# shivams15/navierstokessolver

Hardware: AMD Instinct MI355X
Metric: cell-updates/sec (MLUPS) + Poisson iters/sec, 4096^2 grid at 1/2/4/8 GPUs (higher is better)
Workload: dtype f64

## Files before the change

navierstokessolver_amd/csrc/ns_fps.hip:

```cpp
#include <hip/hip_ext.h>
#include <hip/hip_runtime.h>

#include <algorithm>

#include "ns_internal.h"

namespace nsg {

namespace {

struct cplx {
    double x, y;
};
__device__ inline cplx cadd(cplx a, cplx b) { return {a.x + b.x, a.y + b.y}; }
__device__ inline cplx csub(cplx a, cplx b) { return {a.x - b.x, a.y - b.y}; }
__device__ inline cplx cmul(cplx a, cplx b) { return {fma(a.x, b.x, -a.y * b.y), fma(a.x, b.y, a.y * b.x)}; }

__device__ inline double2 ld2(const double* p) { return *reinterpret_cast<const double2*>(p); }
__device__ inline void st2(double* p, double x, double y) { *reinterpret_cast<double2*>(p) = double2{x, y}; }

__device__ constexpr double C16[8] = {1.0, 0.92387953251128675613, 0.70710678118654752440, 0.38268343236508977173,
                                      0.0, -0.38268343236508977173, -0.70710678118654752440, -0.92387953251128675613};
__device__ constexpr double S16[8] = {0.0, 0.38268343236508977173, 0.70710678118654752440, 0.92387953251128675613,
                                      1.0, 0.92387953251128675613, 0.70710678118654752440, 0.38268343236508977173};
// ... 807 lines not shown
        } else {
#pragma unroll
            for (int q = 0; q < PT; q++) {
                const int k = tid + q * T;
                if (k < N) z[pz(k)] = cplx{ra[q], rb[q]};
            }
            __syncthreads();
            cplx v[PT];
#pragma unroll
            for (int q = 0; q < PT; q++) {
                const int k = tid + q * T;
                if (k < N) {
                    const cplx Xk = z[pz(k)];
                    const cplx Xn = k ? z[pz(N - k)] : cplx{0.0, 0.0};
                    v[q] = conjv(k, Xk.x, Xk.y, Xn.x, Xn.y);
                }
            }
            __syncthreads();
#pragma unroll
            for (int q = 0; q < PT; q++) {
                const int k = tid + q * T;
                if (k < N) z[pz(k)] = v[q];
            }
        }
        __syncthreads();
        fft_lds<LOGN>(z, tw, tid);
        if (PREF && p + (int)gridDim.x < npairs) load(p + gridDim.x);
        double* oa = out + (size_t)r0 * ld;
        double* ob = oa + ld;
#pragma unroll
        for (int q = 0; q < PT; q++) {
            const int j = tid + q * T;
            if (j < N) {
                const int n = (j & 1) ? N - 1 - (j >> 1) : (j >> 1);
                const cplx y = z[pz(n)];
                oa[j] = y.x * rn;
                if (two) ob[j] = -y.y * rn;
            }
        }
        __syncthreads();
    }
}


__device__ inline double piv_next(const FpsArgs& a, int gi, int k, double mu, double rprev, double pw, double pe,
                                  double pem, double& g) {
    const bool oe = a.outE && gi == a.nx - 1;
    g = (oe ? -0.5 * mu : pw) * rprev;
    const double p = fma(-g, pem, oe ? mu : -(pw + pe) + mu);
    return (a.pin && k == 0 && gi == a.nx - 1) ? 0.0 : 1.0 / p;
}


__device__ inline int fps_prow_block(const FpsArgs& a) {
    if (a.prowb) return a.prowb[blockIdx.x];
    return a.ptab && (int)(blockIdx.x * 128) >= a.kfast ? 0 : (1 << 30);
}
__device__ inline void piv_pair(const FpsArgs& a, bool fast, double2 pinf, int gi, int k0, const double (&mu)[2],
                                double (&r)[2], double pw, double pe, double pem, double& g0, double& g1, int pb) {
    if (fast && gi >= pb && gi != a.nx - 1) {
        g0 = pw * r[0];
        g1 = pw * r[1];
        const double2 t = a.ptab && gi < a.prow ? ld2(a.ptab + (size_t)gi * a.ld + k0) : pinf;
        r[0] = t.x;
        r[1] = t.y;
    } else {
        r[0] = piv_next(a, gi, k0, mu[0], r[0], pw, pe, pem, g0);
        r[1] = piv_next(a, gi, k0 + 1, mu[1], r[1], pw, pe, pem, g1);
    }
}

__device__ inline double mode0_shift(const FpsArgs& a, int k0, const double* f = nullptr) {
    if (k0 != 0) return 0.0;
    if (a.outE) return f && !a.s0_given ? 2.0 * f[(size_t)(a.nxl - 1) * a.ld] : *a.s0;
    return a.sh0 ? (a.sh0s != 0.0 ? a.sh0s : (double)a.ny) * *a.sh0 : 0.0;
}
__device__ inline double2 ldf0(const FpsArgs& a, const double* f, int li, int k0, double s0) {
    double2 x = ld2(f + (size_t)li * a.ld + k0);
    x.x -= s0;
    return x;
}

struct ChunkRows {
    double pw[FPS_M], pe[FPS_M], pem[FPS_M];
    __device__ inline void load(const FpsArgs& a, int li0, int rows) {
        (void)rows;
#pragma unroll
        for (int t = 0; t < FPS_M; t++) {
            const int gi = a.i0 + min(li0 + t, a.nxl - 1);
            pw[t] = a.pw[gi];
            pe[t] = a.pe[gi];
            const double pm = a.pe[max(gi - 1, 0)];
            pem[t] = gi > 0 ? pm : 0.0;
        }
    }
    __device__ inline void load_wave(const FpsArgs& a, int li0) {
        if constexpr (3 * FPS_M > 64) {
            load(a, li0, FPS_M);
            return;
        }
        const int lane = threadIdx.x & 63, t = lane % FPS_M, kind = lane / FPS_M;
        const int gi = a.i0 + min(li0 + t, a.nxl - 1);
        const int gk = kind == 2 ? max(gi - 1, 0) : gi;
        const double* src = kind == 0 ? a.pw : a.pe;
        double v = kind < 3 ? src[gk] : 0.0;
        if (kind == 2 && gi == 0) v = 0.0;
        const int lo = __double2loint(v), hi = __double2hiint(v);
        auto rd = [&](int l) {
            return __hiloint2double(__builtin_amdgcn_readlane(hi, l), __builtin_amdgcn_readlane(lo, l));
        };
#pragma unroll
        for (int q = 0; q < FPS_M; q++) {
            pw[q] = rd(q);
            pe[q] = rd(FPS_M + q);
            pem[q] = rd(2 * FPS_M + q);
        }
    }
};

__global__ void __launch_bounds__(64 * FPS_G) k_fps_t1(FpsArgs a, const double* __restrict__ f) {
    __shared__ double2 sE[FPS_G][64], sP[FPS_G][64];
    const int lane = threadIdx.x, w = __builtin_amdgcn_readfirstlane(threadIdx.y);
    const int k0 = 2 * (blockIdx.x * 64 + lane);
    const int grp = blockIdx.y, c = grp * FPS_G + w;
    const int li0 = c * FPS_M;
    const int rows = k0 < a.ny ? min(FPS_M, a.nxl - li0) : 0;
    double E[2] = {0.0, 0.0}, P[2] = {1.0, 1.0};
    if (rows > 0) {
        const double mu[2] = {a.mu[k0], a.mu[k0 + 1]};
        const double2 r0 = ld2(a.rp0 + (size_t)c * a.ld + k0);
        const double s0 = mode0_shift(a, k0);
        ChunkRows cr;
        cr.load(a, li0, rows);
        double2 fv[FPS_M];
#pragma unroll
        for (int t = 0; t < FPS_M; t++)
            if (t < rows) fv[t] = ldf0(a, f, li0 + t, k0, s0);
        double r[2] = {r0.x, r0.y};
#pragma unroll
        for (int t = 0; t < FPS_M; t++) {
            if (t < rows) {
                const int gi = a.i0 + li0 + t;
                const double fm[2] = {fv[t].x, fv[t].y};
#pragma unroll
                for (int m = 0; m < 2; m++) {
                    double g;
                    r[m] = piv_next(a, gi, k0 + m, mu[m], r[m], cr.pw[t], cr.pe[t], cr.pem[t], g);
                    E[m] = fma(-g, E[m], fm[m]);
                    P[m] = -g * P[m];
                }
            }
        }
        st2(a.ca + (size_t)c * a.ld + k0, E[0], E[1]);
        st2(a.ca + (size_t)(a.nch + c) * a.ld + k0, P[0], P[1]);
    }
    sE[w][lane] = double2{E[0], E[1]};
    sP[w][lane] = double2{P[0], P[1]};
    __syncthreads();
    if (w == 0 && k0 < a.ny) {
        double GE[2] = {0.0, 0.0}, GP[2] = {1.0, 1.0};
        for (int q = 0; q < FPS_G; q++) {
            const double2 e = sE[q][lane], pp = sP[q][lane];
            GE[0] = fma(pp.x, GE[0], e.x);
            GE[1] = fma(pp.y, GE[1], e.y);
            GP[0] = pp.x * GP[0];
            GP[1] = pp.y * GP[1];
        }
        st2(a.ga + (size_t)grp * a.ld + k0, GE[0], GE[1]);
        st2(a.ga + (size_t)(a.ngrp + grp) * a.ld + k0, GP[0], GP[1]);
    }
}
// ... 236 lines not shown
    const int li0 = c * FPS_M;
    const int rows = k0 < a.ny ? min(FPS_M, a.nxl - li0) : 0;
    double2 bx{0.0, 0.0}, br{1.0, 1.0};
    if (rows > 0) {
        bx = ld2(a.cb + (size_t)c * a.ld + k0);
        br = ld2(a.cb + (size_t)(a.nch + c) * a.ld + k0);
    }
    sX[w][lane] = bx;
    sR[w][lane] = br;
    __syncthreads();
    if (rows <= 0) return;
    ChunkRows cr;
    cr.load(a, li0, rows);
    double2 xv[FPS_M];
#pragma unroll
    for (int t = 0; t < FPS_M; t++)
        if (t < rows) xv[t] = ld2(f + (size_t)(li0 + t) * a.ld + k0);
    const double2 x0 = ld2(a.gx + (size_t)grp * a.ld + k0);
    double X[2] = {x0.x, x0.y};
    for (int q = FPS_G - 1; q > w; q--) {
        const double2 x = sX[q][lane], rr = sR[q][lane];
        X[0] = fma(rr.x, X[0], x.x);
        X[1] = fma(rr.y, X[1], x.y);
    }
    const double mu[2] = {a.mu[k0], a.mu[k0 + 1]};
    const double2 r0 = ld2(a.rp0 + (size_t)c * a.ld + k0);
    double r[2] = {r0.x, r0.y};
    double2 rv[FPS_M];
#pragma unroll
    for (int t = 0; t < FPS_M; t++) {
        if (t < rows) {
            const int gi = a.i0 + li0 + t;
            double g;
            r[0] = piv_next(a, gi, k0, mu[0], r[0], cr.pw[t], cr.pe[t], cr.pem[t], g);
            r[1] = piv_next(a, gi, k0 + 1, mu[1], r[1], cr.pw[t], cr.pe[t], cr.pem[t], g);
            rv[t] = double2{r[0], r[1]};
        }
    }
    double rho[2] = {1.0, 1.0};
#pragma unroll
    for (int t = FPS_M - 1; t >= 0; t--) {
        if (t < rows) {
            rho[0] = -cr.pe[t] * rv[t].x * rho[0];
            rho[1] = -cr.pe[t] * rv[t].y * rho[1];
            st2(f + (size_t)(li0 + t) * a.ld + k0, fma(rho[0], X[0], xv[t].x), fma(rho[1], X[1], xv[t].y));
        }
    }
}


__global__ void __launch_bounds__(64 * FPS_G) k_fps_t1b(FpsArgs a, const double* __restrict__ f) {
    __shared__ double2 sE[FPS_G][64], sP[FPS_G][64];
    const int lane = threadIdx.x, w = __builtin_amdgcn_readfirstlane(threadIdx.y);
    const int k0 = 2 * (blockIdx.x * 64 + lane);
    const int grp = FPS_SNAKE ? (int)gridDim.y - 1 - (int)blockIdx.y : (int)blockIdx.y, c = grp * FPS_G + w;
    const int li0 = c * FPS_M;
    const int rows = k0 < a.ny ? min(FPS_M, a.nxl - li0) : 0;
    double E[2] = {0.0, 0.0}, P[2] = {1.0, 1.0};
    ChunkRows cr;
    cr.load_wave(a, li0);
    if (rows > 0) {
        const double mu[2] = {a.mu[k0], a.mu[k0 + 1]};
        const double2 r0 = ld2(a.rp0 + (size_t)c * a.ld + k0);
        const double s0 = mode0_shift(a, k0, f);
        double2 yv[FPS_M], rv[FPS_M];
#pragma unroll
        for (int t = 0; t < FPS_M; t++)
            yv[t] = ldf0(a, f, min(li0 + t, a.nxl - 1), k0, s0);
        double r[2] = {r0.x, r0.y};
        const int pb = fps_prow_block(a);
        const bool fast = pb < a.nx;
        const double2 pinf = fast ? ld2(a.pinf + k0) : double2{0.0, 0.0};
#pragma unroll
        for (int t = 0; t < FPS_M; t++) {
            if (t < rows) {
                const int gi = a.i0 + li0 + t;
                double g0, g1;
                piv_pair(a, fast, pinf, gi, k0, mu, r, cr.pw[t], cr.pe[t], cr.pem[t], g0, g1, pb);
                E[0] = fma(-g0, E[0], yv[t].x);
                E[1] = fma(-g1, E[1], yv[t].y);
                P[0] = -g0 * P[0];
                P[1] = -g1 * P[1];
                yv[t] = double2{E[0], E[1]};
                rv[t] = double2{r[0], r[1]};
            }
        }
        double xl[2] = {0.0, 0.0};
#pragma unroll
        for (int t = FPS_M - 1; t >= 0; t--) {
            if (t < rows) {
                xl[0] = fma(yv[t].x, rv[t].x, -cr.pe[t] * rv[t].x * xl[0]);
                xl[1] = fma(yv[t].y, rv[t].y, -cr.pe[t] * rv[t].y * xl[1]);
            }
        }
        st2(a.ca + (size_t)c * a.ld + k0, E[0], E[1]);
        st2(a.ca + (size_t)(a.nch + c) * a.ld + k0, P[0], P[1]);
        st2(a.cb + (size_t)c * a.ld + k0, xl[0], xl[1]);
    }
    sE[w][lane] = double2{E[0], E[1]};
    sP[w][lane] = double2{P[0], P[1]};
    __syncthreads();
    if (w == 0 && k0 < a.ny) {
        double GE[2] = {0.0, 0.0}, GP[2] = {1.0, 1.0};
        for (int q = 0; q < FPS_G; q++) {
            const double2 e = sE[q][lane], pp = sP[q][lane];
            GE[0] = fma(pp.x, GE[0], e.x);
            GE[1] = fma(pp.y, GE[1], e.y);
            GP[0] = pp.x * GP[0];
            GP[1] = pp.y * GP[1];
        }
        st2(a.ga + (size_t)grp * a.ld + k0, GE[0], GE[1]);
        st2(a.ga + (size_t)(a.ngrp + grp) * a.ld + k0, GP[0], GP[1]);
    }
}

__global__ void __launch_bounds__(64) k_fps_mid(FpsArgs a, const double* __restrict__ f) {
    const int k0 = 2 * (blockIdx.x * 64 + threadIdx.x);
    const int grp = blockIdx.y;
    if (k0 >= a.ny) return;
    if (a.outE && !a.s0_given && k0 == 0 && grp == 0) *a.s0 = mode0_shift(a, 0, f);
    const double2 y0 = ld2(a.gc + (size_t)grp * a.ld + k0);
    double Y[2] = {y0.x, y0.y};
    double BX[FPS_G][2], BR[FPS_G][2];
    double2 le[FPS_G], lp[FPS_G], lb[FPS_G], lbe[FPS_G], lbr[FPS_G];
#pragma unroll
    for (int w = 0; w < FPS_G; w++) {
        const int c = min(grp * FPS_G + w, a.nch - 1);
        le[w] = ld2(a.ca + (size_t)c * a.ld + k0);
        lp[w] = ld2(a.ca + (size_t)(a.nch + c) * a.ld + k0);
        lb[w] = ld2(a.cb + (size_t)c * a.ld + k0);
        lbe[w] = ld2(a.bt + (size_t)c * a.ld + k0);
        lbr[w] = ld2(a.bt + (size_t)(a.nch + c) * a.ld + k0);
    }
#pragma unroll
    for (int w = 0; w < FPS_G; w++) {
        const int c = grp * FPS_G + w;
        BX[w][0] = BX[w][1] = 0.0;
        BR[w][0] = BR[w][1] = 1.0;
        if (c < a.nch) {
            double2 e = le[w];
            const double2 pp = lp[w];
            double2 bl = lb[w];
            if (a.m0e && k0 == 0) {
                const double sft = a.ny * *a.m0s;
                e.x -= sft * a.m0e[c];
                bl.x -= sft * a.m0b[c];
            }
            const double2 be = lbe[w], br = lbr[w];
            if (!a.mid_local) st2(a.ya + (size_t)c * a.ld + k0, Y[0], Y[1]);
            BX[w][0] = fma(be.x, Y[0], bl.x);
            BX[w][1] = fma(be.y, Y[1], bl.y);
            BR[w][0] = br.x;
            BR[w][1] = br.y;
            if (!a.mid_local) st2(a.cb + (size_t)c * a.ld + k0, BX[w][0], BX[w][1]);
            Y[0] = fma(pp.x, Y[0], e.x);
            Y[1] = fma(pp.y, Y[1], e.y);
        }
    }
    double GX[2] = {0.0, 0.0}, GR[2] = {1.0, 1.0};
#pragma unroll
    for (int w = FPS_G - 1; w >= 0; w--) {
        GX[0] = fma(BR[w][0], GX[0], BX[w][0]);
        GX[1] = fma(BR[w][1], GX[1], BX[w][1]);
        GR[0] = BR[w][0] * GR[0];
        GR[1] = BR[w][1] * GR[1];
    }
    st2(a.gb + (size_t)grp * a.ld + k0, GX[0], GX[1]);
    st2(a.gb + (size_t)(a.ngrp + grp) * a.ld + k0, GR[0], GR[1]);
}

constexpr int MS_MB = 16;
constexpr int MS_NT = 512;
template <int S, bool BACK, class LE, class LP, class SC>
__device__ __forceinline__ void ms_scan(int ngrp, int ny, int kb, int tid, LE ldE, LP ldP, SC stC, double (*sE)[MS_MB],
                                        double (*sP)[MS_MB], double (*sY)[MS_MB]) {
    const int lane = tid % MS_MB, s = tid / MS_MB;
    const int k = kb + lane;
    constexpr int B = 8;
    auto gq = [&](int q) { return BACK ? ngrp - 1 - q : q; };
    if (S > 1 && ngrp >= 2 * S) {
        const bool act = s < S && k < ny;
        const int per = (ngrp + S - 1) / S, q0 = s * per, q1 = min(ngrp, q0 + per);
        double AE = 0.0, AP = 1.0;
        if (act) {
            for (int qb = q0; qb < q1; qb += B) {
// ... 41 lines not shown
                    const int q = qb + t;
                    if (q < q1) {
                        stC(gq(q), lane, Y);
                        Y = fma(P[t], Y, E[t]);
                    }
                }
            }
        }
    } else if (s == 0 && k < ny) {
        double Y = 0.0;
        for (int q0 = 0; q0 < ngrp; q0 += B) {
            double E[B], P[B];
#pragma unroll
            for (int t = 0; t < B; t++) {
                const int q = q0 + t, qc = min(q, ngrp - 1);
                const double e = ldE(gq(qc), lane), pv = ldP(gq(qc), lane);
                E[t] = q < ngrp ? e : 0.0;
                P[t] = q < ngrp ? pv : 1.0;
            }
#pragma unroll
            for (int t = 0; t < B; t++) {
                const int q = q0 + t;
                if (q < ngrp) {
                    stC(gq(q), lane, Y);
                    Y = fma(P[t], Y, E[t]);
                }
            }
        }
    }
}
template <int S>
__global__ void __launch_bounds__(MS_NT) k_fps_midscan(FpsArgs a, const double* __restrict__ f) {
    extern __shared__ double ms_lds[];
    __shared__ double sE[S][MS_MB], sP[S][MS_MB], sY[S][MS_MB];
    static_assert(MS_NT >= S * MS_MB, "k_fps_midscan: a thread per mode and segment");
    const int tid = threadIdx.x, ngrp = a.ngrp, ld = a.ld, kb = blockIdx.x * MS_MB;
    double* gc = ms_lds;
    double* gbx = gc + (size_t)ngrp * MS_MB;
    double* gbr = gbx + (size_t)ngrp * MS_MB;
    ms_scan<S, false>(
        ngrp, a.ny, kb, tid, [&](int grp, int lane) { return a.ga[(size_t)grp * ld + kb + lane]; },
        [&](int grp, int lane) { return a.ga[(size_t)(ngrp + grp) * ld + kb + lane]; },
        [&](int grp, int lane, double Y) { gc[grp * MS_MB + lane] = Y; }, sE, sP, sY);
    __syncthreads();
    constexpr int NP = MS_MB / 2;
    for (int task = tid; task < NP * ngrp; task += MS_NT) {
        const int pr = task % NP, grp = task / NP;
        const int k0 = kb + 2 * pr;
        if (k0 >= a.ny) continue;
        if (a.outE && !a.s0_given && k0 == 0 && grp == 0) *a.s0 = mode0_shift(a, 0, f);
        double Y[2] = {gc[grp * MS_MB + 2 * pr], gc[grp * MS_MB + 2 * pr + 1]};
        double BX[FPS_G][2], BR[FPS_G][2];
        double2 le[FPS_G], lp[FPS_G], lb[FPS_G], lbe[FPS_G], lbr[FPS_G];
#pragma unroll
        for (int w = 0; w < FPS_G; w++) {
            const int c = min(grp * FPS_G + w, a.nch - 1);
            le[w] = ld2(a.ca + (size_t)c * a.ld + k0);
            lp[w] = ld2(a.ca + (size_t)(a.nch + c) * a.ld + k0);
            lb[w] = ld2(a.cb + (size_t)c * a.ld + k0);
            lbe[w] = ld2(a.bt + (size_t)c * a.ld + k0);
            lbr[w] = ld2(a.bt + (size_t)(a.nch + c) * a.ld + k0);
        }
#pragma unroll
        for (int w = 0; w < FPS_G; w++) {
            const int c = grp * FPS_G + w;
            BX[w][0] = BX[w][1] = 0.0;
            BR[w][0] = BR[w][1] = 1.0;
            if (c < a.nch) {
                double2 e = le[w];
                const double2 pp = lp[w];
                double2 bl = lb[w];
                if (a.m0e && k0 == 0) {
                    const double sft = a.ny * *a.m0s;
                    e.x -= sft * a.m0e[c];
                    bl.x -= sft * a.m0b[c];
                }
                const double2 be = lbe[w], br = lbr[w];
                st2(a.ya + (size_t)c * a.ld + k0, Y[0], Y[1]);
                BX[w][0] = fma(be.x, Y[0], bl.x);
                BX[w][1] = fma(be.y, Y[1], bl.y);
                BR[w][0] = br.x;
                BR[w][1] = br.y;
                st2(a.cb + (size_t)c * a.ld + k0, BX[w][0], BX[w][1]);
                Y[0] = fma(pp.x, Y[0], e.x);
                Y[1] = fma(pp.y, Y[1], e.y);
            }
        }
        double GX[2] = {0.0, 0.0}, GR[2] = {1.0, 1.0};
#pragma unroll
        for (int w = FPS_G - 1; w >= 0; w--) {
            GX[0] = fma(BR[w][0], GX[0], BX[w][0]);
            GX[1] = fma(BR[w][1], GX[1], BX[w][1]);
            GR[0] = BR[w][0] * GR[0];
            GR[1] = BR[w][1] * GR[1];
        }
        gbx[grp * MS_MB + 2 * pr] = GX[0];
        gbx[grp * MS_MB + 2 * pr + 1] = GX[1];
        gbr[grp * MS_MB + 2 * pr] = GR[0];
        gbr[grp * MS_MB + 2 * pr + 1] = GR[1];
    }
    __syncthreads();
    ms_scan<S, true>(
        ngrp, a.ny, kb, tid, [&](int grp, int lane) { return gbx[grp * MS_MB + lane]; },
        [&](int grp, int lane) { return gbr[grp * MS_MB + lane]; },
        [&](int grp, int lane, double Y) { a.gx[(size_t)grp * ld + kb + lane] = Y; }, sE, sP, sY);
}

template <bool GHOST>
__global__ void __launch_bounds__(64 * FPS_G) k_fps_t2b(FpsArgs a, double* __restrict__ f) {
    const int lane = threadIdx.x, w = __builtin_amdgcn_readfirstlane(threadIdx.y);
    const int k0 = 2 * (blockIdx.x * 64 + lane);
    const int grp = blockIdx.y, c = grp * FPS_G + w;
    const int li0 = c * FPS_M;
    const int rows = k0 < a.ny ? min(FPS_M, a.nxl - li0) : 0;
    ChunkRows cr;
    cr.load_wave(a, li0);
    if (rows <= 0) return;
    const double s0 = mode0_shift(a, k0);
    double2 yv[FPS_M];
#pragma unroll
    for (int t = 0; t < FPS_M; t++)
        yv[t] = ldf0(a, f, min(li0 + t, a.nxl - 1), k0, s0);
    const double2 yin = ld2(a.ya + (size_t)c * a.ld + k0);
    const double2 x0 = ld2(a.gx + (size_t)grp * a.ld + k0);
    double X[2] = {x0.x, x0.y};
    for (int q = FPS_G - 1; q > w; q--) {
        const int cq = grp * FPS_G + q;
        if (cq >= a.nch) continue;
        const double2 bx = ld2(a.cb + (size_t)cq * a.ld + k0), br = ld2(a.bt + (size_t)(a.nch + cq) * a.ld + k0);
        X[0] = fma(br.x, X[0], bx.x);
        X[1] = fma(br.y, X[1], bx.y);
    }
    if (GHOST && c == a.nch - 1 && a.i0 + a.nxl < a.nx) st2(f + (size_t)a.nxl * a.ld + k0, X[0], X[1]);
    const double mu[2] = {a.mu[k0], a.mu[k0 + 1]};
    const double2 r0 = ld2(a.rp0 + (size_t)c * a.ld + k0);
    double r[2] = {r0.x, r0.y}, y[2] = {yin.x, yin.y};
    double2 rv[FPS_M];
    const int pb = fps_prow_block(a);
    const bool fast = pb < a.nx;
    const double2 pinf = fast ? ld2(a.pinf + k0) : double2{0.0, 0.0};
#pragma unroll
    for (int t = 0; t < FPS_M; t++) {
        if (t < rows) {
            const int gi = a.i0 + li0 + t;
            double g0, g1;
            piv_pair(a, fast, pinf, gi, k0, mu, r, cr.pw[t], cr.pe[t], cr.pem[t], g0, g1, pb);
            y[0] = fma(-g0, y[0], yv[t].x);
            y[1] = fma(-g1, y[1], yv[t].y);
            yv[t] = double2{y[0], y[1]};
            rv[t] = double2{r[0], r[1]};
        }
    }
#pragma unroll
    for (int t = FPS_M - 1; t >= 0; t--) {
        if (t < rows) {
            X[0] = fma(yv[t].x, rv[t].x, -cr.pe[t] * rv[t].x * X[0]);
            X[1] = fma(yv[t].y, rv[t].y, -cr.pe[t] * rv[t].y * X[1]);
            st2(f + (size_t)(li0 + t) * a.ld + k0, X[0], X[1]);
        }
    }
    if (GHOST && c == 0 && a.i0 > 0) {
        const double2 yi = ld2(a.ya + k0), rq = ld2(a.rp0 + k0);
        const double pe = a.pe[a.i0 - 1];
        st2(f - (ptrdiff_t)a.ld + k0, fma(yi.x, rq.x, -pe * rq.x * X[0]), fma(yi.y, rq.y, -pe * rq.y * X[1]));
    }
}

bool fps_div_real(const Knobs& k, int logn, int outE);
template <int LOGN>
void idct_row(const double* in, double* out, int nrows, int ld, const void* tw, const void* wk, hipStream_t st) {
    const size_t lr = sizeof(cplx) * (size_t)RFft<LOGN>::M;
    lds_attr_once((const void*)k_fps_idct_r<LOGN>, (int)lr);
    hipEvent_t a, b;
    if (take_launch_timing(a, b))
        hipExtLaunchKernelGGL(k_fps_idct_r<LOGN>, dim3(nrows), dim3(RFft<LOGN>::T), lr, st, a, b, 0, in, out, nrows,
                              ld, (const cplx*)tw, (const cplx*)wk);
    else
        hipLaunchKernelGGL(k_fps_idct_r<LOGN>, dim3(nrows), dim3(RFft<LOGN>::T), lr, st, in, out, nrows, ld,
                           (const cplx*)tw, (const cplx*)wk);
}
template <int LOGN>
void dct_pair(const Knobs& k, bool inverse, const double* in, const double* shift, double* out, int nrows, int ld, const void* tw,
              const void* wk, hipStream_t st, int oe_pair, const int32_t* fcm = nullptr) {
    constexpr int T = Fft<LOGN>::T;
    const size_t lds = sizeof(cplx) * (size_t)FftLds<LOGN>::n;
    const dim3 grid(std::min((nrows + 1) / 2, k.fps_grid > 0 ? k.fps_grid : 1 << 30));
    if constexpr (LOGN >= 10 && LOGN <= 13) {
        if (inverse && !fcm && fps_div_real(k, LOGN, 0)) {
            idct_row<LOGN>(in, out, nrows, ld, tw, wk, st);
            return;
        }
// ... 675 lines not shown
```

navierstokessolver_amd/csrc/ns_internal.h:

```cpp
#pragma once
#include <hip/hip_runtime.h>
#include <cstdint>
#include <vector>

#include "ns_knobs.h"

#ifndef NS_TAILS
#define NS_TAILS 1
#endif

namespace nsg {

constexpr int HALO = 7;

constexpr int FC_IN = 1 << 20;
constexpr int FC_DEEP = 1 << 21;
constexpr int FC_BAND = 1 << 22;
constexpr int FC_INT = 31;
constexpr int MAX_EDGES = 31;
__host__ __device__ inline int fc_edge(int code, int k) { return (code >> (5 * k)) & 31; }
struct EdgeDev {
    int neu;
    int enx, eny;
    double c0, c1;
};

struct Geo {
    const int32_t* fc = nullptr;
    const EdgeDev* et = nullptr;
    int nx, ny;
    int i0, nxl;
    int ld;
    int neu[4];
    double c0[4], c1[4];
    int enx[4], eny[4];
    int sr0 = 0, sr1 = 1 << 30;
    int dsx = 0;
    const int* ecell = nullptr;
    int necell = 0;
};

struct Coef {
    const double *hx, *hy;
    const double *pw, *pe, *ps, *pn;
    const double *bx, *by;
    const double *rhx, *rhy;
    const double *rsx, *rsy;
    const double *fwx, *fex, *fsy, *fny;
    int yuni = 0;
};

struct Partials {
    double* p;
    int n;
};

int launch_rhs(const Knobs& kn, const Geo& g, const Coef& c, double dt, double re, const double* u, const double* v,
               const double* phi, double* cu, double* cv, double* ru, double* rv, double* part, hipStream_t st,
               int depth = 2, double* uo = nullptr, double* vo = nullptr, double* mm = nullptr);
struct Buoy {
    double bx, by, tref;
// ... 123 lines not shown
    int rows;
};
int launch_helm_rb_mask(const Geo& g, const Coef& c, double alpha, double omega, double* x, const double* b,
                        double* x2, const double* b2, int par, double* part, hipStream_t st);
constexpr int MT_TI = 32, MT_TJ = 64;
int launch_helm_mt_mask(const Geo& g, const Coef& c, double alpha, double omega, const double* u, const double* v,
                        const double* bu, const double* bv, double* uo, double* vo, int nsw, double* part,
                        hipStream_t st, const double* qbu = nullptr, const double* qbv = nullptr,
                        const int* tiles = nullptr, int ntiles = 0);
void launch_helm_rbt_mask(const Geo& g, const Coef& c, double alpha, double omega, const double* u, const double* v,
                          const double* bu, const double* bv, double* uo, double* vo, hipStream_t st);
int launch_apply(const Knobs& kn, int op, const Geo& g, const Coef& c, double alpha, const double* x, double* y, const double* q,
                 double* part, hipStream_t st, const double* stop = nullptr);
void launch_diag_pc(int op, const Geo& g, const Coef& c, double alpha, const double* q, double* z, hipStream_t st,
                    const double* stop = nullptr);
int launch_bicg_vec(int mode, KrylovArgs a, hipStream_t st);
void launch_bicg_scal(int stage, const double* d, double n, double* sc, hipStream_t st);
void launch_bicg_start(double* sc, double thr, double b2, int maxit, hipStream_t st);

int max_partials(const Geo& g);

#ifndef FPS_ROWS
#define FPS_ROWS 16
#endif
constexpr int FPS_M = FPS_ROWS;
#ifndef FPS_GRP
#define FPS_GRP 4
#endif
constexpr int FPS_G = FPS_GRP;
constexpr int FPS_LOGN_MIN = 4;
constexpr int FPS_LOGN_MAX = 13;
struct FpsArgs {
    int nx, i0, nxl, ny, ld;
    int nch, ngrp;
    int pin;
    const double *pw, *pe;
    const double* mu;
    const double* rp0;
    double* ca;
    double *ga, *gc;
    double *gb, *gx;
    double* cb;
    const double* bt;
    double* ya;
    const double* sh0 = nullptr;
    double sh0s = 0.0;
    const double *m0e = nullptr, *m0b = nullptr, *m0s = nullptr;
    int outE = 0;
    double* s0 = nullptr;
    int s0_given = 0;
    const double *ptab = nullptr, *pinf = nullptr;
    int prow = 0, kfast = 1 << 30;
    const int* prowb = nullptr;
    int mid_local = 0;
    int ghost = 0;
};
struct FpsRank {
    const double* gath = nullptr;
    int P = 1, r = 0, stride = 0;
    const double *a1 = nullptr, *ge1 = nullptr;
    double ncells = 0.0;
    double* shift = nullptr;
    const double *bq = nullptr, *x1 = nullptr;
};
int fps_log2(int ny);
bool fps_idct_mask_ok(int ny);
bool fps_fuse_ok(const Knobs& kn, int ny, int outE);
int launch_fps_idct_masked(const Knobs& kn, const double* in, double* out, int nrows, int ny, int ld, const double* tw, const double* wk,
                           hipStream_t st, const int32_t* fcm);
int launch_fps_dct(const Knobs& kn, bool inverse, const double* in, const double* shift, double* out, int nrows, int ny, int ld,
                   const double* tw, const double* wk, hipStream_t st, int oe_pair = -1, const double* tw8 = nullptr);
int fps_log2x(int ny);
bool fps_gen_ok(int ny);
void launch_dense_mats(const double* C, const double* shy, double rsum, int N, double* F, double* G, hipStream_t st);
int launch_fps_div(const Knobs& kn, const Geo& g, const Coef& c, double dt, const double* u, const double* v, double* b, double* out,
                   double* part, int phase, const double* tw, const double* wk, hipStream_t st, int outE = 0);
void launch_fps_t1(const FpsArgs& a, const double* f, hipStream_t st);
void launch_fps_t2(const FpsArgs& a, double* f, hipStream_t st);
void launch_fps_t3(const FpsArgs& a, double* f, hipStream_t st);
void launch_fps_t1b(const FpsArgs& a, const double* f, hipStream_t st);
void launch_fps_mid(const FpsArgs& a, const double* f, hipStream_t st);
bool launch_fps_midscan(const FpsArgs& a, const double* f, hipStream_t st);
void launch_fps_t2b(const FpsArgs& a, double* f, hipStream_t st);
void launch_fps_oe_s0(const double* f, int row, int ld, int last, double* out, hipStream_t st);
void launch_fps_scan(const FpsArgs& a, bool backward, const FpsRank& R, double* rout, hipStream_t st);

struct CapArgs {
    int m = 0, ncell = 0, border = 0;
    const double* e1 = nullptr;
    const int *fi = nullptr, *fj = nullptr, *fk = nullptr, *fm = nullptr, *co = nullptr;
    const int4* cf = nullptr;
    const double* w = nullptr;
    double *cinv = nullptr, *y = nullptr;
};
constexpr size_t CAP_LDS_MAX = 8192;
hipError_t launch_cap_gemv(const CapArgs& a, const double* z, hipStream_t st);
void launch_cap_scatter(const CapArgs& a, double* q, int mode, hipStream_t st);
void launch_cap_axpy(const Geo& g, const CapArgs& a, double* x, const double* z, int set, hipStream_t st);
void launch_cap_fill(const Geo& g, double* q, double val, hipStream_t st);
void launch_cap_rhs(const Geo& g, const double* b, const double* shift, double* r, hipStream_t st);
void launch_cap_src(const CapArgs& a, double* q, int fprev, int f, hipStream_t st);
void launch_cap_col(const CapArgs& a, const double* z, int f, double* cmat, hipStream_t st);
void launch_gj_invert(double* A, int m, double* t, double* u, double* flag, int spd, hipStream_t st);

}
```

navierstokessolver_amd/csrc/ns_solver.cpp:

```cpp
#include <rccl/rccl.h>
#include <rocblas/rocblas.h>
#include <rocsolver/rocsolver.h>
#include <dlfcn.h>
#include <limits>

#include <algorithm>
#include <cmath>
#include <cstdarg>
#include <cstdio>
#include <cstring>
#include <map>
#include <string>
#include <vector>

#include "../../include/nsgpu.h"
#include "ns_internal.h"

namespace {

thread_local std::string g_err;

void set_err(const char* fmt, ...) {
    char buf[1024];
    va_list ap;
// ... 2160 lines not shown
                    if (conv[k] < 0 && !left[k] && gi > 1 && fixed) conv[k] = gi;
                    if (mode == 2 && conv[k] >= 0 && rn != rr[k]) {
                        conv[k] = -1;
                        left[k] = 1;
                    }
                    rr[k] = rn;
                    if (mode == 1) ptab[(size_t)gi * ld + k] = rn;
                }
            }
            if (mode == 2) {
                const int nb = (ld + 127) / 128;
                prowb.assign(nb, 1 << 30);
                bool any = false;
                for (int b = 0; b < nb; b++) {
                    int mx = 0;
                    bool ok = b * 128 < N;
                    for (int k = b * 128; k < std::min(N, (b + 1) * 128) && ok; k++) {
                        ok = conv[k] >= 0;
                        mx = std::max(mx, conv[k]);
                    }
                    if (ok) { prowb[b] = mx + 1; any = true; }
                }
                if (any) {
                    pinf.assign(ld, 0.0);
                    for (int k = 0; k < N; k++) pinf[k] = rr[k];
                } else {
                    prowb.clear();
                }
            } else {
            for (int kf = 128; kf < N; kf += 128) {
                int mx = 0;
                bool ok = true;
                for (int k = kf; k < N && ok; k++) {
                    ok = conv[k] >= 0;
                    mx = std::max(mx, conv[k]);
                }
                if (ok) {
                    kfast = kf;
                    prow = std::min(PRMAX, (mx + 1 + 15) / 16 * 16);
                    break;
                }
            }
            if (kfast < N) {
                pinf.assign(ld, 0.0);
                for (int k = 0; k < N; k++) pinf[k] = rr[k];
                ptab.resize((size_t)prow * ld);
            } else {
                ptab.clear();
                kfast = 1 << 30;
            }
            }
        }
    }
    const size_t n_pt = !ptab.empty() ? ptab.size() + (size_t)ld : (!prowb.empty() ? (size_t)ld + prowb.size() : 0);
    const size_t n_t8 = nsg::fps_log2(N) < 0 ? (size_t)N : 0;
    HIPCHK(hipMalloc(&s->fps_mem, (total + n_pt + n_t8) * sizeof(double)));
    HIPCHK(hipMemset(s->fps_mem, 0, (total + n_pt + n_t8) * sizeof(double)));
    HIPCHK(hipMemcpy(s->fps_mem, h.data(), h.size() * sizeof(double), hipMemcpyHostToDevice));
    if (n_t8) {
        std::vector<double> t8(n_t8);
        for (int m = 0; m < N / 2; m++) {
            t8[2 * m] = h[4 * m];
            t8[2 * m + 1] = h[4 * m + 1];
        }
        s->fps_tw8 = s->fps_mem + total + n_pt;
        HIPCHK(hipMemcpy(s->fps_mem + total + n_pt, t8.data(), n_t8 * sizeof(double), hipMemcpyHostToDevice));
    }
    if (n_pt && !ptab.empty()) {
        double* pt = s->fps_mem + total;
        HIPCHK(hipMemcpy(pt, ptab.data(), ptab.size() * sizeof(double), hipMemcpyHostToDevice));
        HIPCHK(hipMemcpy(pt + ptab.size(), pinf.data(), (size_t)ld * sizeof(double), hipMemcpyHostToDevice));
        a.ptab = pt;
        a.pinf = pt + ptab.size();
        a.prow = prow;
        a.kfast = kfast;
    } else if (n_pt) {
        double* pt = s->fps_mem + total;
        HIPCHK(hipMemcpy(pt, pinf.data(), (size_t)ld * sizeof(double), hipMemcpyHostToDevice));
        int* pb = reinterpret_cast<int*>(pt + ld);
        HIPCHK(hipMemcpy(pb, prowb.data(), prowb.size() * sizeof(int), hipMemcpyHostToDevice));
        a.pinf = pt;
        a.prowb = pb;
    }
    double* d = s->fps_mem;
    s->fps_tw = d;
    s->fps_wk = d + 2 * (size_t)N;
    a.mu = d + 4 * (size_t)N;
    a.rp0 = d + n_tab;
    a.bt = d + n_tab + n_rp0;
    double* q = d + n_tab + n_rp0 + n_bt;
    a.ga = q; q += 2 * n_g;
    a.gc = q; q += n_g;
    a.gb = q; q += 2 * n_g;
    a.gx = q; q += n_g;
    a.cb = q; q += 2 * (size_t)nchp * ld;
    a.ca = q; q += 2 * (size_t)nchp * ld;
    a.ya = q; q += (size_t)nchp * ld;
    a.s0 = d + total - 8;
    if (n_mr) {
        s->fps_ragg = q; q += s->fps_n;
        s->fps_gath = q; q += (size_t)s->nranks * s->fps_n;
        const int nx = g.nx;
        std::vector<double> r0(nx);
        {
            double rp = 0.0;
            for (int gi = 0; gi < nx; gi++) {
                const double gg = pw[gi] * rp, pem = gi > 0 ? pe[gi - 1] : 0.0;
                const double p = std::fma(-gg, pem, -(pw[gi] + pe[gi]) + 0.0);
                rp = r0[gi] = gi == nx - 1 ? 0.0 : 1.0 / p;
            }
        }
        auto fwd = [&](int ga, int gb) {
            double E = 0.0;
            for (int gi = ga; gi < gb; gi++) E = std::fma(-(pw[gi] * (gi > 0 ? r0[gi - 1] : 0.0)), E, 1.0);
            return E;
        };
        std::vector<double> m0((size_t)2 * nchp + a.ngrp + s->nranks, 0.0);
        for (int c = 0; c < a.nch; c++) {
            const int gi0 = g.i0 + c * nsg::FPS_M, gi1 = std::min(gi0 + nsg::FPS_M, g.i0 + g.nxl);
            std::vector<double> y;
            double E = 0.0;
            for (int gi = gi0; gi < gi1; gi++) {
                E = std::fma(-(pw[gi] * (gi > 0 ? r0[gi - 1] : 0.0)), E, 1.0);
                y.push_back(E);
            }
            double xl = 0.0;
            for (int gi = gi1 - 1; gi >= gi0; gi--) xl = std::fma(y[gi - gi0], r0[gi], -pe[gi] * r0[gi] * xl);
            m0[c] = E;
            m0[(size_t)nchp + c] = xl;
        }
        for (int gq = 0; gq < a.ngrp; gq++)
            m0[2 * (size_t)nchp + gq] = fwd(g.i0 + gq * nsg::FPS_G * nsg::FPS_M,
                                            std::min(g.i0 + (gq + 1) * nsg::FPS_G * nsg::FPS_M, g.i0 + g.nxl));
        for (int rq = 0; rq < s->nranks; rq++) {
            int32_t q0, q1;
            ns_slab_range(g.nx, s->nranks, rq, &q0, &q1);
            m0[2 * (size_t)nchp + a.ngrp + rq] = fwd(q0, q1);
        }
        HIPCHK(hipMemcpy(q, m0.data(), m0.size() * sizeof(double), hipMemcpyHostToDevice));
        s->m0e = q;
        s->m0b = q + nchp;
        s->m0g = q + 2 * (size_t)nchp;
        s->m0a = s->m0g + a.ngrp;
        q += m0.size();
        if (s->fps_og) {
            const int P = s->nranks;
            std::vector<double> B((size_t)P * ld, 0.0), X1(P, 0.0), rr(N, 0.0), fw(N), bw(N);
            int rq = 0;
            int32_t q0 = 0, q1 = 0;
            ns_slab_range(nx, P, 0, &q0, &q1);
            double y1 = 0.0, bw1 = 1.0;
            for (int gi = 0; gi < nx; gi++) {
                while (gi >= q1) { rq++; ns_slab_range(nx, P, rq, &q0, &q1); }
                if (gi == q0) {
                    std::fill(fw.begin(), fw.end(), 1.0);
                    std::fill(bw.begin(), bw.end(), 1.0);
                    y1 = 0.0;
                    bw1 = 1.0;
                }
                const double pem = gi > 0 ? pe[gi - 1] : 0.0;
                double* Bq = B.data() + (size_t)rq * ld;
                const bool oe = a.outE && gi == nx - 1;
                for (int k = 0; k < N; k++) {
                    const double gg = (oe ? -0.5 * h[4 * N + k] : pw[gi]) * rr[k];
                    const double p = std::fma(-gg, pem, oe ? h[4 * N + k] : -(pw[gi] + pe[gi]) + h[4 * N + k]);
                    rr[k] = (k == 0 && gi == nx - 1) ? 0.0 : 1.0 / p;
                    fw[k] *= -gg;
                    Bq[k] += fw[k] * rr[k] * bw[k];
                    bw[k] *= -pe[gi] * rr[k];
                }
                y1 = std::fma(-(pw[gi] * (gi > 0 ? r0[gi - 1] : 0.0)), y1, 1.0);
                X1[rq] += y1 * r0[gi] * bw1;
                bw1 *= -pe[gi] * r0[gi];
            }
            HIPCHK(hipMemcpy(q, B.data(), B.size() * sizeof(double), hipMemcpyHostToDevice));
            s->og_b = q;
            q += B.size();
            HIPCHK(hipMemcpy(q, X1.data(), X1.size() * sizeof(double), hipMemcpyHostToDevice));
            s->og_x1 = q;
            q += X1.size();
        }
    }
    a.pw = s->c.pw;
    a.pe = s->c.pe;
    return 0;
}

std::vector<double> coef_tables(const std::vector<double>& hx, const std::vector<double>& hy,
                                const int* neu = nullptr) {
    const int nz[4] = {0, 0, 0, 0};
    if (!neu) neu = nz;
    const int nx = (int)hx.size(), ny = (int)hy.size();
    std::vector<double> h(8 * (size_t)nx + 8 * (size_t)ny + 2, 0.0);
    double *pw = h.data(), *pe = pw + nx, *bx = pe + nx, *ps = bx + nx, *pn = ps + ny, *by = pn + ny;
    double *hxo = by + ny, *hyo = hxo + nx;
    double *rhx = hyo + ny, *rhy = rhx + nx, *rsx = rhy + ny, *rsy = rsx + nx + 1;
    double *fwx = rsy + ny + 1, *fex = fwx + nx, *fsy = fex + nx, *fny = fsy + ny;
    for (int i = 0; i < nx; i++) {
        fwx[i] = i > 0 ? hx[i] / (hx[i - 1] + hx[i]) : 0.0;
        fex[i] = i < nx - 1 ? hx[i] / (hx[i + 1] + hx[i]) : 0.0;
    }
    for (int j = 0; j < ny; j++) {
        fsy[j] = j > 0 ? hy[j] / (hy[j - 1] + hy[j]) : 0.0;
        fny[j] = j < ny - 1 ? hy[j] / (hy[j + 1] + hy[j]) : 0.0;
    }
    for (int i = 0; i < nx; i++) rhx[i] = 1.0 / hx[i];
    for (int j = 0; j < ny; j++) rhy[j] = 1.0 / hy[j];
    for (int i = 1; i < nx; i++) rsx[i] = 2.0 / (hx[i - 1] + hx[i]);
    for (int j = 1; j < ny; j++) rsy[j] = 2.0 / (hy[j - 1] + hy[j]);
    for (int i = 0; i < nx; i++) {
        const double a = hx[i];
        hxo[i] = a;
        pw[i] = i > 0 ? 2.0 / (a * (a + hx[i - 1])) : 0.0;
        pe[i] = i < nx - 1 ? 2.0 / (a * (a + hx[i + 1])) : 0.0;
        bx[i] = (i == 0 && !neu[0] ? 2.0 / (a * a) : 0.0) + (i == nx - 1 && !neu[1] ? 2.0 / (a * a) : 0.0);
    }
    for (int j = 0; j < ny; j++) {
        const double a = hy[j];
        hyo[j] = a;
        ps[j] = j > 0 ? 2.0 / (a * (a + hy[j - 1])) : 0.0;
        pn[j] = j < ny - 1 ? 2.0 / (a * (a + hy[j + 1])) : 0.0;
        by[j] = (j == 0 && !neu[2] ? 2.0 / (a * a) : 0.0) + (j == ny - 1 && !neu[3] ? 2.0 / (a * a) : 0.0);
    }
    return h;
}

nsg::Coef coef_view(double* d, int nx, int ny) {
    nsg::Coef c{};
    c.pw = d; c.pe = d + nx; c.bx = d + 2 * nx;
    c.ps = d + 3 * nx; c.pn = d + 3 * nx + ny; c.by = d + 3 * nx + 2 * ny;
    c.hx = d + 3 * nx + 3 * ny; c.hy = d + 4 * nx + 3 * ny;
    c.rhx = d + 4 * nx + 4 * ny; c.rhy = d + 5 * nx + 4 * ny;
    c.rsx = d + 5 * nx + 5 * ny; c.rsy = d + 6 * nx + 5 * ny + 1;
    c.fwx = d + 6 * nx + 6 * ny + 2; c.fex = c.fwx + nx; c.fsy = c.fex + nx; c.fny = c.fsy + ny;
    return c;
}

// ... 1975 lines not shown
```

Measured before the change: 15480.

## Skip pivot recurrences for chunks where tridiagonal pivots have reached a fixed point

In the FFT-Poisson tridiagonal solve, the setup now finds chunks (per 128-mode block) whose coefficients are uniform and whose pivots have already converged to pinf. For those chunks, t1b and t2b run a simplified recurrence with constant g and q and skip loading per-row coefficients and pivots. The aggregate kernels read one shared fixed P/bt row instead of per-chunk rows. Blocks are also remapped so that block column 0 (the slow, non-fixed one) is scheduled first. This only applies to single-rank, non-outflow cases, and it depends on exact bitwise equality checks done on the host at setup.

```diff
diff --git a/navierstokessolver_amd/csrc/ns_fps.hip b/navierstokessolver_amd/csrc/ns_fps.hip
--- a/navierstokessolver_amd/csrc/ns_fps.hip
+++ b/navierstokessolver_amd/csrc/ns_fps.hip
@@ -883,9 +883,9 @@
 }
 
 
-__device__ inline int fps_prow_block(const FpsArgs& a) {
-    if (a.prowb) return a.prowb[blockIdx.x];
-    return a.ptab && (int)(blockIdx.x * 128) >= a.kfast ? 0 : (1 << 30);
+__device__ inline int fps_prow_block(const FpsArgs& a, int b = blockIdx.x) {
+    if (a.prowb) return a.prowb[b];
+    return a.ptab && (int)(b * 128) >= a.kfast ? 0 : (1 << 30);
 }
 __device__ inline void piv_pair(const FpsArgs& a, bool fast, double2 pinf, int gi, int k0, const double (&mu)[2],
                                 double (&r)[2], double pw, double pe, double pem, double& g0, double& g1, int pb) {
@@ -948,6 +948,27 @@
         }
     }
 };
+
+__device__ inline bool fps_chunk_fixed(const FpsArgs& a, int c, int b = blockIdx.x) {
+    if (!NS_FPS_FIXED || !a.cfix) return false;
+    return c <= a.clast && c >= a.cfix[b];
+}
+__device__ inline bool fps_group_fixed(const FpsArgs& a, int b, int grp) {
+    if (!NS_FPS_FIXED || !a.cfix) return false;
+    return grp * FPS_G + FPS_G - 1 <= a.clast && grp * FPS_G >= a.cfix[b];
+}
+
+__device__ inline void fps_block0_first(const FpsArgs& a, int& bx, int& by) {
+    if (!NS_FPS_FIXED || !a.cfix || gridDim.x < 2) return;
+    const int nbx = gridDim.x, ng = gridDim.y, L = by * nbx + bx;
+    if (L < ng) {
+        bx = 0;
+        by = L;
+    } else {
+        bx = 1 + (L - ng) % (nbx - 1);
+        by = (L - ng) / (nbx - 1);
+    }
+}
 
 __global__ void __launch_bounds__(64 * FPS_G) k_fps_t1(FpsArgs a, const double* __restrict__ f) {
     __shared__ double2 sE[FPS_G][64], sP[FPS_G][64];
@@ -1290,11 +1311,42 @@
 __global__ void __launch_bounds__(64 * FPS_G) k_fps_t1b(FpsArgs a, const double* __restrict__ f) {
     __shared__ double2 sE[FPS_G][64], sP[FPS_G][64];
     const int lane = threadIdx.x, w = __builtin_amdgcn_readfirstlane(threadIdx.y);
-    const int k0 = 2 * (blockIdx.x * 64 + lane);
-    const int grp = FPS_SNAKE ? (int)gridDim.y - 1 - (int)blockIdx.y : (int)blockIdx.y, c = grp * FPS_G + w;
+    int bx = blockIdx.x, by = blockIdx.y;
+    fps_block0_first(a, bx, by);
+    const int k0 = 2 * (bx * 64 + lane);
+    const int grp = FPS_SNAKE ? (int)gridDim.y - 1 - by : by, c = grp * FPS_G + w;
     const int li0 = c * FPS_M;
     const int rows = k0 < a.ny ? min(FPS_M, a.nxl - li0) : 0;
     double E[2] = {0.0, 0.0}, P[2] = {1.0, 1.0};
+    if (fps_chunk_fixed(a, c, bx)) {
+        if (rows > 0) {
+            const double s0 = mode0_shift(a, k0, f);
+            double2 yv[FPS_M];
+#pragma unroll
+            for (int t = 0; t < FPS_M; t++) yv[t] = ldf0(a, f, li0 + t, k0, s0);
+            const double2 pinf = ld2(a.pinf + k0);
+            const double pw = a.pw[a.i0 + li0], pe = a.pe[a.i0 + li0];
+            const double g0 = pw * pinf.x, g1 = pw * pinf.y;
+            const double q0 = -pe * pinf.x, q1 = -pe * pinf.y;
+#pragma unroll
+            for (int t = 0; t < FPS_M; t++) {
+                E[0] = fma(-g0, E[0], yv[t].x);
+                E[1] = fma(-g1, E[1], yv[t].y);
+                P[0] = -g0 * P[0];
+                P[1] = -g1 * P[1];
+                yv[t] = double2{E[0], E[1]};
+            }
+            double xl[2] = {0.0, 0.0};
+#pragma unroll
+            for (int t = FPS_M - 1; t >= 0; t--) {
+                xl[0] = fma(yv[t].x, pinf.x, q0 * xl[0]);
+                xl[1] = fma(yv[t].y, pinf.y, q1 * xl[1]);
+            }
+            st2(a.ca + (size_t)c * a.ld + k0, E[0], E[1]);
+            if (!(a.fixv && fps_group_fixed(a, bx, grp))) st2(a.ca + (size_t)(a.nch + c) * a.ld + k0, P[0], P[1]);
+            st2(a.cb + (size_t)c * a.ld + k0, xl[0], xl[1]);
+        }
+    } else {
     ChunkRows cr;
     cr.load_wave(a, li0);
     if (rows > 0) {
@@ -1306,7 +1358,7 @@
         for (int t = 0; t < FPS_M; t++)
             yv[t] = ldf0(a, f, min(li0 + t, a.nxl - 1), k0, s0);
         double r[2] = {r0.x, r0.y};
-        const int pb = fps_prow_block(a);
+        const int pb = fps_prow_block(a, bx);
         const bool fast = pb < a.nx;
         const double2 pinf = fast ? ld2(a.pinf + k0) : double2{0.0, 0.0};
 #pragma unroll
@@ -1335,6 +1387,7 @@
         st2(a.ca + (size_t)(a.nch + c) * a.ld + k0, P[0], P[1]);
         st2(a.cb + (size_t)c * a.ld + k0, xl[0], xl[1]);
     }
+    }
     sE[w][lane] = double2{E[0], E[1]};
     sP[w][lane] = double2{P[0], P[1]};
     __syncthreads();
@@ -1361,14 +1414,29 @@
     double Y[2] = {y0.x, y0.y};
     double BX[FPS_G][2], BR[FPS_G][2];
     double2 le[FPS_G], lp[FPS_G], lb[FPS_G], lbe[FPS_G], lbr[FPS_G];
+    const bool gf = a.fixv && fps_group_fixed(a, blockIdx.x, grp);
 #pragma unroll
     for (int w = 0; w < FPS_G; w++) {
         const int c = min(grp * FPS_G + w, a.nch - 1);
         le[w] = ld2(a.ca + (size_t)c * a.ld + k0);
-        lp[w] = ld2(a.ca + (size_t)(a.nch + c) * a.ld + k0);
         lb[w] = ld2(a.cb + (size_t)c * a.ld + k0);
-        lbe[w] = ld2(a.bt + (size_t)c * a.ld + k0);
-        lbr[w] = ld2(a.bt + (size_t)(a.nch + c) * a.ld + k0);
+    }
+    if (gf) {
+        const double2 fp = ld2(a.fixv + k0), fbe = ld2(a.fixv + (size_t)a.ld + k0), fbr = ld2(a.fixv + 2 * (size_t)a.ld + k0);
+#pragma unroll
+        for (int w = 0; w < FPS_G; w++) {
+            lp[w] = fp;
+            lbe[w] = fbe;
+            lbr[w] = fbr;
+        }
+    } else {
+#pragma unroll
+        for (int w = 0; w < FPS_G; w++) {
+            const int c = min(grp * FPS_G + w, a.nch - 1);
+            lp[w] = ld2(a.ca + (size_t)(a.nch + c) * a.ld + k0);
+            lbe[w] = ld2(a.bt + (size_t)c * a.ld + k0);
+            lbr[w] = ld2(a.bt + (size_t)(a.nch + c) * a.ld + k0);
+        }
     }
 #pragma unroll
     for (int w = 0; w < FPS_G; w++) {
@@ -1516,14 +1584,29 @@
         double Y[2] = {gc[grp * MS_MB + 2 * pr], gc[grp * MS_MB + 2 * pr + 1]};
         double BX[FPS_G][2], BR[FPS_G][2];
         double2 le[FPS_G], lp[FPS_G], lb[FPS_G], lbe[FPS_G], lbr[FPS_G];
+        const bool gf = a.fixv && fps_group_fixed(a, k0 / 128, grp);
 #pragma unroll
         for (int w = 0; w < FPS_G; w++) {
             const int c = min(grp * FPS_G + w, a.nch - 1);
             le[w] = ld2(a.ca + (size_t)c * a.ld + k0);
-            lp[w] = ld2(a.ca + (size_t)(a.nch + c) * a.ld + k0);
             lb[w] = ld2(a.cb + (size_t)c * a.ld + k0);
-            lbe[w] = ld2(a.bt + (size_t)c * a.ld + k0);
-            lbr[w] = ld2(a.bt + (size_t)(a.nch + c) * a.ld + k0);
+        }
+        if (gf) {
+            const double2 fp = ld2(a.fixv + k0), fbe = ld2(a.fixv + (size_t)a.ld + k0), fbr = ld2(a.fixv + 2 * (size_t)a.ld + k0);
+#pragma unroll
+            for (int w = 0; w < FPS_G; w++) {
+                lp[w] = fp;
+                lbe[w] = fbe;
+                lbr[w] = fbr;
+            }
+        } else {
+#pragma unroll
+            for (int w = 0; w < FPS_G; w++) {
+                const int c = min(grp * FPS_G + w, a.nch - 1);
+                lp[w] = ld2(a.ca + (size_t)(a.nch + c) * a.ld + k0);
+                lbe[w] = ld2(a.bt + (size_t)c * a.ld + k0);
+                lbr[w] = ld2(a.bt + (size_t)(a.nch + c) * a.ld + k0);
+            }
         }
 #pragma unroll
         for (int w = 0; w < FPS_G; w++) {
@@ -1573,10 +1656,48 @@
 template <bool GHOST>
 __global__ void __launch_bounds__(64 * FPS_G) k_fps_t2b(FpsArgs a, double* __restrict__ f) {
     const int lane = threadIdx.x, w = __builtin_amdgcn_readfirstlane(threadIdx.y);
-    const int k0 = 2 * (blockIdx.x * 64 + lane);
-    const int grp = blockIdx.y, c = grp * FPS_G + w;
+    int bx = blockIdx.x, by = blockIdx.y;
+    if (!GHOST) fps_block0_first(a, bx, by);
+    const int k0 = 2 * (bx * 64 + lane);
+    const int grp = by, c = grp * FPS_G + w;
     const int li0 = c * FPS_M;
     const int rows = k0 < a.ny ? min(FPS_M, a.nxl - li0) : 0;
+    if (!GHOST && fps_chunk_fixed(a, c, bx)) {
+        if (rows <= 0) return;
+        const double s0 = mode0_shift(a, k0);
+        double2 yv[FPS_M];
+#pragma unroll
+        for (int t = 0; t < FPS_M; t++) yv[t] = ldf0(a, f, li0 + t, k0, s0);
+        const double2 yin = ld2(a.ya + (size_t)c * a.ld + k0);
+        const double2 x0 = ld2(a.gx + (size_t)grp * a.ld + k0);
+        double X[2] = {x0.x, x0.y};
+        for (int q = FPS_G - 1; q > w; q--) {
+            const int cq = grp * FPS_G + q;
+            if (cq >= a.nch) continue;
+            const double* brp = a.fixv && cq <= a.clast ? a.fixv + 2 * (size_t)a.ld : a.bt + (size_t)(a.nch + cq) * a.ld;
+            const double2 bx = ld2(a.cb + (size_t)cq * a.ld + k0), br = ld2(brp + k0);
+            X[0] = fma(br.x, X[0], bx.x);
+            X[1] = fma(br.y, X[1], bx.y);
+        }
+        const double2 pinf = ld2(a.pinf + k0);
+        const double pw = a.pw[a.i0 + li0], pe = a.pe[a.i0 + li0];
+        const double g0 = pw * pinf.x, g1 = pw * pinf.y;
+        const double q0 = -pe * pinf.x, q1 = -pe * pinf.y;
+        double y[2] = {yin.x, yin.y};
+#pragma unroll
+        for (int t = 0; t < FPS_M; t++) {
+            y[0] = fma(-g0, y[0], yv[t].x);
+            y[1] = fma(-g1, y[1], yv[t].y);
+            yv[t] = double2{y[0], y[1]};
+        }
+#pragma unroll
+        for (int t = FPS_M - 1; t >= 0; t--) {
+            X[0] = fma(yv[t].x, pinf.x, q0 * X[0]);
+            X[1] = fma(yv[t].y, pinf.y, q1 * X[1]);
+            st2(f + (size_t)(li0 + t) * a.ld + k0, X[0], X[1]);
+        }
+        return;
+    }
     ChunkRows cr;
     cr.load_wave(a, li0);
     if (rows <= 0) return;
@@ -1600,7 +1721,7 @@
     const double2 r0 = ld2(a.rp0 + (size_t)c * a.ld + k0);
     double r[2] = {r0.x, r0.y}, y[2] = {yin.x, yin.y};
     double2 rv[FPS_M];
-    const int pb = fps_prow_block(a);
+    const int pb = fps_prow_block(a, bx);
     const bool fast = pb < a.nx;
     const double2 pinf = fast ? ld2(a.pinf + k0) : double2{0.0, 0.0};
 #pragma unroll
diff --git a/navierstokessolver_amd/csrc/ns_internal.h b/navierstokessolver_amd/csrc/ns_internal.h
--- a/navierstokessolver_amd/csrc/ns_internal.h
+++ b/navierstokessolver_amd/csrc/ns_internal.h
@@ -7,6 +7,9 @@
 
 #ifndef NS_TAILS
 #define NS_TAILS 1
+#endif
+#ifndef NS_FPS_FIXED
+#define NS_FPS_FIXED 1
 #endif
 
 namespace nsg {
@@ -236,6 +239,9 @@
     const double *ptab = nullptr, *pinf = nullptr;
     int prow = 0, kfast = 1 << 30;
     const int* prowb = nullptr;
+    const int* cfix = nullptr;
+    int clast = -1;
+    const double* fixv = nullptr;
     int mid_local = 0;
     int ghost = 0;
 };
diff --git a/navierstokessolver_amd/csrc/ns_solver.cpp b/navierstokessolver_amd/csrc/ns_solver.cpp
--- a/navierstokessolver_amd/csrc/ns_solver.cpp
+++ b/navierstokessolver_amd/csrc/ns_solver.cpp
@@ -2236,7 +2236,39 @@
             }
         }
     }
-    const size_t n_pt = !ptab.empty() ? ptab.size() + (size_t)ld : (!prowb.empty() ? (size_t)ld + prowb.size() : 0);
+    std::vector<int> cfix;
+    int clast = -1;
+    int* d_cfix = nullptr;
+    double* d_fixv = nullptr;
+    if (NS_FPS_FIXED && !prowb.empty() && s->nranks == 1 && g.i0 == 0 && g.nxl == g.nx && !a.outE) {
+        const int nb = (int)prowb.size();
+        auto plain = [&](int c) {
+            const int gi0 = c * nsg::FPS_M;
+            if (gi0 < 1 || gi0 + nsg::FPS_M > g.nx - 1) return false;
+            for (int gi = gi0; gi < gi0 + nsg::FPS_M; gi++)
+                if (std::memcmp(&pw[gi], &pw[gi0 - 1], sizeof(double)) || std::memcmp(&pe[gi], &pe[gi0 - 1], sizeof(double)))
+                    return false;
+            return true;
+        };
+        for (int c = a.nch - 1; c >= 0 && clast < 0; c--)
+            if (plain(c)) clast = c;
+        cfix.assign(nb, 1 << 30);
+        long nfix = 0;
+        for (int b = 0; b < nb && clast >= 0; b++) {
+            if (prowb[b] >= g.nx) continue;
+            const int k1 = std::min(N, (b + 1) * 128);
+            for (int c = clast; c >= 0; c--) {
+                bool ok = plain(c) && c * nsg::FPS_M >= prowb[b];
+                for (int k = b * 128; k < k1 && ok; k++)
+                    ok = std::memcmp(&rp0[(size_t)c * ld + k], &pinf[k], sizeof(double)) == 0;
+                if (!ok) break;
+                cfix[b] = c;
+            }
+            if (cfix[b] <= clast) nfix += clast - cfix[b] + 1;
+        }
+        if (nfix == 0) cfix.clear();
+    }
+    const size_t n_pt = !ptab.empty() ? ptab.size() + (size_t)ld : (!prowb.empty() ? (size_t)ld + prowb.size() + 3 * (size_t)ld : 0);
     const size_t n_t8 = nsg::fps_log2(N) < 0 ? (size_t)N : 0;
     HIPCHK(hipMalloc(&s->fps_mem, (total + n_pt + n_t8) * sizeof(double)));
     HIPCHK(hipMemset(s->fps_mem, 0, (total + n_pt + n_t8) * sizeof(double)));
@@ -2261,10 +2293,12 @@
     } else if (n_pt) {
         double* pt = s->fps_mem + total;
         HIPCHK(hipMemcpy(pt, pinf.data(), (size_t)ld * sizeof(double), hipMemcpyHostToDevice));
-        int* pb = reinterpret_cast<int*>(pt + ld);
+        int* pb = reinterpret_cast<int*>(pt + 4 * (size_t)ld);
         HIPCHK(hipMemcpy(pb, prowb.data(), prowb.size() * sizeof(int), hipMemcpyHostToDevice));
         a.pinf = pt;
         a.prowb = pb;
+        d_cfix = pb + prowb.size();
+        d_fixv = pt + ld;
     }
     double* d = s->fps_mem;
     s->fps_tw = d;
@@ -2367,6 +2401,51 @@
     }
     a.pw = s->c.pw;
     a.pe = s->c.pe;
+    long nfix = 0;
+    if (!cfix.empty() && d_cfix) {
+        const size_t npl = (size_t)g.nxl * ld, nP = (size_t)a.nch * ld;
+        double* zero = nullptr;
+        HIPCHK(hipMalloc(&zero, npl * sizeof(double)));
+        HIPCHK(hipMemsetAsync(zero, 0, npl * sizeof(double), s->st));
+        nsg::launch_fps_t1b(a, zero, s->st);
+        std::vector<double> hP(nP);
+        HIPCHK(hipMemcpyAsync(hP.data(), a.ca + nP, nP * sizeof(double), hipMemcpyDeviceToHost, s->st));
+        HIPCHK(hipStreamSynchronize(s->st));
+        HIPCHK(hipFree(zero));
+        std::vector<double> fv(3 * (size_t)ld, 0.0);
+        const double* tab[3] = {hP.data(), bt, bt + nP};
+        for (int b = 0; b < (int)cfix.size(); b++) {
+            if (cfix[b] > clast) continue;
+            const int k0 = b * 128, nk = std::min(N, k0 + 128) - k0;
+            bool ok = true;
+            for (int q = 0; q < 3 && ok; q++) {
+                const double* row0 = tab[q] + (size_t)cfix[b] * ld + k0;
+                std::memcpy(&fv[(size_t)q * ld + k0], row0, nk * sizeof(double));
+                for (int c = cfix[b] + 1; c <= clast && ok; c++)
+                    ok = std::memcmp(tab[q] + (size_t)c * ld + k0, row0, nk * sizeof(double)) == 0;
+            }
+            if (ok) nfix += clast - cfix[b] + 1;
+            else cfix[b] = 1 << 30;
+        }
+        if (nfix > 0) {
+            HIPCHK(hipMemcpy(d_fixv, fv.data(), fv.size() * sizeof(double), hipMemcpyHostToDevice));
+            HIPCHK(hipMemcpy(d_cfix, cfix.data(), cfix.size() * sizeof(int), hipMemcpyHostToDevice));
+            a.cfix = d_cfix;
+            a.clast = clast;
+            a.fixv = d_fixv;
+        }
+    }
+    if (s->k.verbose && s->rank == 0) {
+        const int nbm = (N + 127) / 128;
+        fprintf(stderr, "nsgpu fps: fixed chunks %ld of %ld (block, chunk) pairs", nfix, (long)nbm * a.nch);
+        if (nfix > 0) {
+            fprintf(stderr, " (%d x %d, last fixed chunk %d); fixed-point rows:", nbm, a.nch, clast);
+            for (int b = 0; b < nbm; b++) fprintf(stderr, prowb[b] >= g.nx ? " -" : " %d", prowb[b]);
+            fprintf(stderr, "; first fixed chunks:");
+            for (int b = 0; b < nbm; b++) fprintf(stderr, cfix[b] > clast ? " -" : " %d", cfix[b]);
+        }
+        fprintf(stderr, "\n");
+    }
     return 0;
 }
 
```

Measured after the change: 15740 (median of 6 runs). 1.02x the previous value.
